# serycjon/WOFT

Hardware: AMD Instinct MI355X
Metric: tracked frames/sec at 1080p, 12 RAFT iters; flow EPE vs reference (higher is better)
Workload: dtype bf16x3 (split-bf16 MFMA operands emulating fp32, fp32 accumulate)

## Files before the change

woft_amd/csrc/conv_1x1_band.hip:

```cpp
#include "conv_1x1_tile.h"
#include "lookup_blocks.h"

int woft_conv_check(const woft_conv_params& p);

namespace {

struct BlockRows {
    int py0, px0, hf, wf;
    __device__ __forceinline__ int64_t operator()(int row) const {
        const int y = py0 + (row >> 3), x = px0 + (row & 7);
        return (y < hf && x < wf) ? (int64_t)y * wf + x : -1;
    }
};

template <int TERMS>
struct GeomBand {
    using G = Geom1x1<TERMS, 2>;
    static constexpr int R = 4, NW = 2 * R + 1, N2 = NW * NW, WS = NW + 1, LEVELS = 4;
    static constexpr int RING = 4;
    static constexpr int RS = WOFT_BAND_LD + 4;
    static constexpr int HR = 6, PLD = HR * RS;
    static constexpr int RING_ELEMS = RING * G::A_ELEMS;
    static constexpr int WIN_ELEMS = 64 * PLD * 2;
    static constexpr int SMEM_ELEMS = RING_ELEMS + WIN_ELEMS;
    static_assert(SMEM_ELEMS >= G::STAGE_ELEMS && SMEM_ELEMS >= Geom1x1<TERMS, 1>::SMEM_ELEMS, "one LDS array for every phase");
    static_assert((RING_ELEMS * 2) % 16 == 0, "the windows start 16-byte aligned");
};

template <int TERMS>
__global__ __launch_bounds__(256, 2) void conv1x1_band_kernel(const woft_conv_params pa, const woft_conv_params pb,
                                                              const woft_lookup_band_params bp, const int split) {
    using GB = GeomBand<TERMS>;
    using G = Geom1x1<TERMS, 2>;
    constexpr int NP = G::NP, TM = G::TM, TN = 2, A_PLANE = G::A_PLANE, A_ELEMS = G::A_ELEMS, WCOLS = G::WCOLS;
    constexpr int R = GB::R, NW = GB::NW, WS = GB::WS, RS = GB::RS, PLD = GB::PLD, NT = 256, NB = 4, NCHUNK = 11;
    constexpr int STEP_ELEMS = NP * 2 * 64 * 8;
    __shared__ __attribute__((aligned(16))) __bf16 smem[GB::SMEM_ELEMS];
    __shared__ int s_ox[GB::LEVELS][64], s_oy[GB::LEVELS][64];
    __shared__ float s_fx[GB::LEVELS][64], s_fy[GB::LEVELS][64];

    if ((int)blockIdx.x >= split) {
        int m_tile, n_tile;
        woft::tile_of_block((int)blockIdx.x - split, m_tiles_1x1(pb), pb.cout_pad / 128, m_tile, n_tile);
        tile_1x1<TERMS, 1, true, 4, 4>(pb, m_tile, n_tile, smem);
        return;
    }
    const woft_lookup_otf_params& p = bp.otf;
    __bf16* const ring = smem;
    float* const Wl = (float*)(smem + GB::RING_ELEMS);

    const int tid = threadIdx.x;
    const int lane = tid & 63;
    const int wave = __builtin_amdgcn_readfirstlane(tid >> 6);
    const int r32 = lane & 31, hh = lane >> 5;
    const int tiles_x = (p.wf + 7) / 8;
    int tile;
    {
        const int q = split / 8, rr = split % 8, xcd = blockIdx.x % 8, idx = blockIdx.x / 8;
        tile = (xcd < rr ? xcd * (q + 1) : rr * (q + 1) + (xcd - rr) * q) + idx;
    }
    const int px0 = (tile % tiles_x) * 8, py0 = (tile / tiles_x) * 8;

    const __bf16* wstream[TN];
#pragma unroll
    for (int j = 0; j < TN; ++j) wstream[j] = (const __bf16*)pa.wgt_frag + (int64_t)(wave * TN + j) * NCHUNK * STEP_ELEMS + lane * 8;
    bf16x8 bq[NB][TN][NP];
    auto fetch_b = [&](int step, auto slot_tag) {
        constexpr int slot = decltype(slot_tag)::value;
        const int s = step < 2 * NCHUNK ? step : 2 * NCHUNK - 1;
        const int off = (s >> 1) * STEP_ELEMS + (s & 1) * 512;
#pragma unroll
        for (int j = 0; j < TN; ++j)
#pragma unroll
            for (int pl = 0; pl < NP; ++pl) bq[slot][j][pl] = *(const bf16x8*)(wstream[j] + off + pl * 1024);
    };
    [&]<int... S>(std::integer_sequence<int, S...>) {
        (fetch_b(S, std::integral_constant<int, S>{}), ...);
    }(std::make_integer_sequence<int, NB - 1>{});

    int ok = 1;
    {
        const int y = py0 + (lane >> 3), x = px0 + (lane & 7);
        const bool cvalid = tid < 64 && y < p.hf && x < p.wf;
        if (cvalid) {
            const int64_t i = (int64_t)y * p.wf + x;
            const float cx = p.coords[i * 2], cy = p.coords[i * 2 + 1];
#pragma unroll
            for (int l = 0; l < GB::LEVELS; ++l) {
                const float sc = 1.0f / (float)(1 << l);
                const float xs = cx * sc, ys = cy * sc;
                float flx = floorf(xs), fly = floorf(ys);
                s_fx[l][tid] = xs - flx;
                s_fy[l][tid] = ys - fly;
                flx = fminf(fmaxf(flx, -1.0e6f), 1.0e6f);
                fly = fminf(fmaxf(fly, -1.0e6f), 1.0e6f);
                const int m = WOFT_BAND_M(l);
                const int ox = (int)flx - (x >> l) + m, oy = (int)fly - (y >> l) + m;
                ok &= (ox >= 0 && ox <= 2 * m && oy >= 0 && oy <= 2 * m) ? 1 : 0;
                s_ox[l][tid] = ox;
                s_oy[l][tid] = oy;
            }
        } else if (tid < 64) {
#pragma unroll
            for (int l = 0; l < GB::LEVELS; ++l) {
                s_fx[l][tid] = s_fy[l][tid] = 0.f;
                s_ox[l][tid] = s_oy[l][tid] = 0;
            }
        }
    }
    const bool hit = __builtin_amdgcn_readfirstlane(__syncthreads_and(ok)) != 0;

    constexpr int ROWS = 16 + 14 + 12 + 12;
    f32x4 pc[GB::HR];
    auto load_half = [&](auto l_tag, auto h_tag) __attribute__((always_inline)) {
        constexpr int l = decltype(l_tag)::value, half = decltype(h_tag)::value;
        constexpr int NR = half == 0 ? 6 : 5, R0 = half == 0 ? 0 : 5;
        constexpr int roff = l == 0 ? 0 : (l == 1 ? 16 : (l == 2 ? 30 : 42));
        static_assert(64 * NR * 4 == NR * NT, "NR pieces per thread");
#pragma unroll
        for (int k = 0; k < NR; ++k) {
            const int it = tid + k * NT;
            const int pix = it / (4 * NR), rem = it - pix * (4 * NR);
            const int gy = py0 + (pix >> 3), gx = px0 + (pix & 7);
            pc[k] = f32x4{0.f, 0.f, 0.f, 0.f};
            if (gy < p.hf && gx < p.wf) {
                const int ox = s_ox[l][pix];
                pc[k] = *(const f32x4*)(bp.band + (((int64_t)gy * p.wf + gx) * ROWS + roff + ox + R0) * WOFT_BAND_LD + rem * 4);
            }
        }
    };
    auto store_half = [&](auto h_tag) __attribute__((always_inline)) {
        constexpr int half = decltype(h_tag)::value;
        constexpr int NR = half == 0 ? 6 : 5;
#pragma unroll
        for (int k = 0; k < NR; ++k) {
            const int it = tid + k * NT;
            const int pix = it / (4 * NR), rem = it - pix * (4 * NR);
            *(f32x4*)(Wl + pix * PLD + (rem >> 2) * RS + (rem & 3) * 4) = pc[k];
        }
    };
    auto sample = [&](auto l_tag, int pix, int c, int lrow) __attribute__((always_inline)) {
        constexpr int l = decltype(l_tag)::value;
        const int gy = py0 + (pix >> 3), gx = px0 + (pix & 7);
        if (gy >= p.hf || gx >= p.wf) return;
        const float fx = s_fx[l][pix], fy = s_fy[l][pix];
        const float* cq = Wl + pix * PLD + lrow * RS + s_oy[l][pix];
        float h[WS];
#pragma unroll
        for (int j = 0; j < WS; ++j) h[j] = cq[j] * (1.f - fx) + cq[RS + j] * fx;
        float o[12];
#pragma unroll
        for (int j = 0; j < NW; ++j) o[j] = h[j] * (1.f - fy) + h[j + 1] * fy;
        o[9] = o[10] = o[11] = 0.f;
        const int ch0 = l * GB::N2 + c * NW;
#pragma unroll
        for (int g = 0; g < 3; ++g) {
            const f32x4 val = {o[4 * g], o[4 * g + 1], o[4 * g + 2], o[4 * g + 3]};
            const bf16x4 hi = cvt16<TERMS>(val);
            bf16x4 lo = hi;
            if (NP == 2) lo = __builtin_convertvector(val - widen_bf16x4(hi), bf16x4);
#pragma unroll
            for (int e = 0; e < 4; ++e) {
                if (4 * g + e >= NW) continue;
                const int ch = ch0 + 4 * g + e;
                __bf16* a = ring + ((ch >> 5) & (GB::RING - 1)) * A_ELEMS + pix * LDB + (ch & 31);
                a[0] = hi[e];
                if (NP == 2) a[A_PLANE] = lo[e];
            }
        }
    };
    const int row = tid >> 2, v = tid & 3;
    const int64_t mrow = BlockRows{py0, px0, p.hf, p.wf}(row);
    auto fill_chunk = [&](int chunk) __attribute__((always_inline)) {
        const f32x4 zero = {0.f, 0.f, 0.f, 0.f};
        f32x4 rh[2] = {zero, zero};
        if (mrow >= 0) {
            const uint32_t off = (uint32_t)mrow * (uint32_t)pa.cs0 + (uint32_t)(chunk * BK + 8 * v);
            rh[0] = *(const f32x4*)(pa.in0 + off);
            rh[1] = *(const f32x4*)(pa.in0 + off + 4);
        }
        bf16x4 hi[2], lo[2];
#pragma unroll
        for (int e = 0; e < 2; ++e) {
            hi[e] = cvt16<TERMS>(rh[e]);
            if (NP == 2) lo[e] = __builtin_convertvector(rh[e] - widen_bf16x4(hi[e]), bf16x4);
        }
        __bf16* As = ring + (chunk & (GB::RING - 1)) * A_ELEMS;
        *(bf16x8*)(As + row * LDB + 8 * v) = __builtin_shufflevector(hi[0], hi[1], 0, 1, 2, 3, 4, 5, 6, 7);
        if (NP == 2) *(bf16x8*)(As + A_PLANE + row * LDB + 8 * v) = __builtin_shufflevector(lo[0], lo[1], 0, 1, 2, 3, 4, 5, 6, 7);
    };

    f32x16 acc[TM][TN];
#pragma unroll
    for (int i = 0; i < TM; ++i)
#pragma unroll
        for (int j = 0; j < TN; ++j)
#pragma unroll
            for (int r = 0; r < 16; ++r) acc[i][j][r] = 0.f;
    const int a_off = r32 * LDB + hh * 8;
    auto run_chunk = [&](auto c_tag) __attribute__((always_inline)) {
        constexpr int c = decltype(c_tag)::value;
        const __bf16* As = ring + (c & (GB::RING - 1)) * A_ELEMS;
        bf16x8 aq[2][TM][NP];
#pragma unroll
        for (int s2 = 0; s2 < 2; ++s2)
#pragma unroll
            for (int i = 0; i < TM; ++i)
#pragma unroll
                for (int pl = 0; pl < NP; ++pl) aq[s2][i][pl] = *(const bf16x8*)(As + a_off + i * 32 * LDB + pl * A_PLANE + s2 * 16);
        [&]<int... S2>(std::integer_sequence<int, S2...>) {
            ([&] {
                constexpr int s2 = S2, slot = (2 * c + s2) % NB;
                fetch_b(2 * c + s2 + NB - 1, std::integral_constant<int, (2 * c + s2 + NB - 1) % NB>{});
                __builtin_amdgcn_sched_barrier(0);
                if (NP == 2) {
#pragma unroll
                    for (int j = 0; j < TN; ++j)
#pragma unroll
                        for (int i = 0; i < TM; ++i) acc[i][j] = mma16<TERMS>(aq[s2][i][NP - 1], bq[slot][j][0], acc[i][j]);
#pragma unroll
                    for (int j = 0; j < TN; ++j)
#pragma unroll
                        for (int i = 0; i < TM; ++i) acc[i][j] = mma16<TERMS>(aq[s2][i][0], bq[slot][j][NP - 1], acc[i][j]);
                }
#pragma unroll
                for (int j = 0; j < TN; ++j)
#pragma unroll
                    for (int i = 0; i < TM; ++i) acc[i][j] = mma16<TERMS>(aq[s2][i][0], bq[slot][j][0], acc[i][j]);
                __builtin_amdgcn_sched_barrier(0);
            }(), ...);
        }(std::make_integer_sequence<int, 2>{});
    };

    if (hit) load_half(std::integral_constant<int, 0>{}, std::integral_constant<int, 0>{});
    auto level = [&](auto l_tag) __attribute__((always_inline)) {
        constexpr int l = decltype(l_tag)::value;
        constexpr int c_first = l == 0 ? 0 : (l == 1 ? 2 : (l == 2 ? 5 : 7));
        constexpr int c_last = l == 0 ? 1 : (l == 1 ? 4 : (l == 2 ? 6 : 10));
        static_assert(c_last == (l == 3 ? NCHUNK - 1 : ((l + 1) * GB::N2) / BK - 1) && c_last - c_first < GB::RING, "ring of four chunk tiles");
        if (hit) {
            store_half(std::integral_constant<int, 0>{});
            __syncthreads();
            load_half(l_tag, std::integral_constant<int, 1>{});
            if (l == 3) {
                __bf16* As = ring + ((NCHUNK - 1) & (GB::RING - 1)) * A_ELEMS + row * LDB;
                const bf16x4 z4 = __builtin_bit_cast(bf16x4, (uint64_t)0);
#pragma unroll
                for (int pl = 0; pl < NP; ++pl) {
                    if (v == 0) *(bf16x4*)(As + pl * A_PLANE + 4) = z4;
                    else *(bf16x8*)(As + pl * A_PLANE + 8 * v) = __builtin_shufflevector(z4, z4, 0, 1, 2, 3, 4, 5, 6, 7);
                }
            }
            for (int it = tid; it < 64 * 5; it += NT) {
                const int pix = it / 5, c = it - pix * 5;
                sample(l_tag, pix, c, c);
            }
            __syncthreads();
            store_half(std::integral_constant<int, 1>{});
            __syncthreads();
            if constexpr (l + 1 < GB::LEVELS) load_half(std::integral_constant<int, l + 1>{}, std::integral_constant<int, 0>{});
            sample(l_tag, tid >> 2, 5 + (tid & 3), tid & 3);
        } else {
            __syncthreads();
#pragma unroll
            for (int c = c_first; c <= c_last; ++c) fill_chunk(c);
        }
        __syncthreads();
        [&]<int... C>(std::integer_sequence<int, C...>) {
            (run_chunk(std::integral_constant<int, c_first + C>{}), ...);
        }(std::make_integer_sequence<int, c_last - c_first + 1>{});
    };
    level(std::integral_constant<int, 0>{});
    level(std::integral_constant<int, 1>{});
    level(std::integral_constant<int, 2>{});
    level(std::integral_constant<int, 3>{});
    __syncthreads();
    woft::conv_epilogue_t<TM, TN, G::BM, WCOLS, G::ST>(pa, acc, (float*)smem + wave * G::ST * woft::STAGE_FLOATS,
                                                        BlockRows{py0, px0, p.hf, p.wf}, 0, 0, wave, lane, tile);
}

}

extern "C" int woft_conv1x1_band(const woft_conv_params* c1, const woft_conv_params* f1, const woft_lookup_band_params* bp,
                                 void* stream) {
    if (c1 == nullptr || bp == nullptr || bp->band == nullptr) return WOFT_EINVAL;
    const woft_lookup_otf_params& o = bp->otf;
    if (o.radius != 4 || o.k != 256 || o.levels != 4 || (o.terms != 1 && o.terms != 3) || o.coords == nullptr || o.out == nullptr ||
        o.hf <= 0 || o.wf <= 0 || o.need != nullptr || o.ablate != 0)
        return WOFT_EINVAL;
    if ((o.roi_y0 | o.roi_x0 | o.roi_h | o.roi_w | o.smp_y0 | o.smp_x0 | o.smp_h | o.smp_w) != 0) return WOFT_EINVAL;
    for (const woft_conv_params* q : {c1, f1}) {
        if (q == nullptr) continue;
        if (woft_conv_check(*q) != WOFT_OK) return WOFT_EINVAL;
        const woft_conv_params& p = *q;
        if (p.halo != 16 || p.precision < 1 || p.precision > 3 || p.precision != c1->precision) return WOFT_EINVAL;
        if (p.stride != 1 || p.ho != p.h || p.wo != p.w || p.taps_x != 1) return WOFT_EINVAL;
        if (p.wgt_frag == nullptr || p.stat_sum != nullptr || p.in_norm != 0 || p.wh0_lookup != nullptr) return WOFT_EINVAL;
        if (p.epi == WOFT_EPI_FLOWHEAD || p.epi == WOFT_EPI_WH_MEAN || p.epi == WOFT_EPI_CTX) return WOFT_EINVAL;
        if ((p.roi_y0 | p.roi_x0 | p.roi_h | p.roi_w) != 0) return WOFT_EINVAL;
        const int64_t cs_max = (p.in1 != nullptr && p.cs1 > p.cs0) ? p.cs1 : p.cs0;
        if ((int64_t)p.n_img * p.h * p.w * cs_max >= (1ll << 31)) return WOFT_EINVAL;
    }
    if (c1->flat || c1->taps_y != 1 || c1->pad_y != 0 || c1->pad_x != 0 || c1->tile_n != 256 || c1->cin_pad != 352 ||
        c1->cout_pad != 256 || c1->in1 != nullptr || c1->n_img != 1 || c1->h != o.hf || c1->w != o.wf)
        return WOFT_EINVAL;
    if (c1->in0 != o.out || c1->cs0 != o.ldo || o.ldo < 352) return WOFT_EINVAL;
    if (f1 != nullptr && (!f1->flat || f1->cin_pad != 32 || f1->tile_n != 128 || 2 * f1->pad_y + 1 != f1->taps_y ||
                          f1->cout_pad % 128 != 0))
        return WOFT_EINVAL;
    const int split = ((o.hf + 7) / 8) * ((o.wf + 7) / 8);
    const int64_t extra = f1 != nullptr ? (int64_t)m_tiles_1x1(*f1) * (f1->cout_pad / 128) : 0;
    dim3 grid((unsigned)(split + extra));
    hipStream_t s = (hipStream_t)stream;
    const woft_conv_params& pb = f1 != nullptr ? *f1 : *c1;
    switch (c1->precision) {
        case 1: woft_launch(0, conv1x1_band_kernel<3>, grid, dim3(256), 0, s, *c1, pb, *bp, split); break;
        case 2: woft_launch(0, conv1x1_band_kernel<1>, grid, dim3(256), 0, s, *c1, pb, *bp, split); break;
        default: woft_launch(0, conv1x1_band_kernel<16>, grid, dim3(256), 0, s, *c1, pb, *bp, split); break;
    }
    return woft_launch_status();
}
```

Before: 130.9.

## Remap band window loads and sampling to one pixel per thread quad

Band-window loads and LDS stores now use a fixed row/quarter mapping per thread (pixel = tid>>2, quarter = tid&3) instead of per-iteration div/mod over pixels. Sampling is re-split so each thread of the quad samples whole rows plus a three-way split of row 4, which removes the loop over 320 items and its idle tail. Per-pixel fx/fy/oy are loaded once per level, and a 31→0 chunk-boundary split handles writes that cross ring tiles. Compile-time-gated timing stamps (WOFT_C1BAND_PROBE) are added but are off by default.

```diff
diff --git a/woft_amd/csrc/conv_1x1_band.hip b/woft_amd/csrc/conv_1x1_band.hip
--- a/woft_amd/csrc/conv_1x1_band.hip
+++ b/woft_amd/csrc/conv_1x1_band.hip
@@ -2,6 +2,19 @@
 #include "lookup_blocks.h"
 
 int woft_conv_check(const woft_conv_params& p);
+
+#ifdef WOFT_C1BAND_PROBE
+#define C1B_STAMPS 46
+#define C1B_STAMP(i, clock)                                      \
+    do {                                                         \
+        __builtin_amdgcn_sched_barrier(0);                       \
+        if (lane == 0) s_stamp[wave][i] = (uint32_t)(clock);     \
+        __builtin_amdgcn_sched_barrier(0);                       \
+    } while (0)
+#else
+#define C1B_STAMP(i, clock) do {} while (0)
+#endif
+#define C1B_TIME(i) C1B_STAMP(i, __builtin_amdgcn_s_memtime())
 
 namespace {
 
@@ -33,11 +46,14 @@
     using GB = GeomBand<TERMS>;
     using G = Geom1x1<TERMS, 2>;
     constexpr int NP = G::NP, TM = G::TM, TN = 2, A_PLANE = G::A_PLANE, A_ELEMS = G::A_ELEMS, WCOLS = G::WCOLS;
-    constexpr int R = GB::R, NW = GB::NW, WS = GB::WS, RS = GB::RS, PLD = GB::PLD, NT = 256, NB = 4, NCHUNK = 11;
+    constexpr int R = GB::R, NW = GB::NW, RS = GB::RS, PLD = GB::PLD, NT = 256, NB = 4, NCHUNK = 11;
     constexpr int STEP_ELEMS = NP * 2 * 64 * 8;
     __shared__ __attribute__((aligned(16))) __bf16 smem[GB::SMEM_ELEMS];
     __shared__ int s_ox[GB::LEVELS][64], s_oy[GB::LEVELS][64];
     __shared__ float s_fx[GB::LEVELS][64], s_fy[GB::LEVELS][64];
+#ifdef WOFT_C1BAND_PROBE
+    __shared__ uint32_t s_stamp[4][C1B_STAMPS];
+#endif
 
     if ((int)blockIdx.x >= split) {
         int m_tile, n_tile;
@@ -52,6 +68,8 @@
     const int tid = threadIdx.x;
     const int lane = tid & 63;
     const int wave = __builtin_amdgcn_readfirstlane(tid >> 6);
+    C1B_STAMP(44, __builtin_amdgcn_s_memrealtime());
+    C1B_TIME(0);
     const int r32 = lane & 31, hh = lane >> 5;
     const int tiles_x = (p.wf + 7) / 8;
     int tile;
@@ -110,67 +128,60 @@
     }
     const bool hit = __builtin_amdgcn_readfirstlane(__syncthreads_and(ok)) != 0;
 
+    const int row = tid >> 2, v = tid & 3;
+    const int64_t mrow = BlockRows{py0, px0, p.hf, p.wf}(row);
+
     constexpr int ROWS = 16 + 14 + 12 + 12;
     f32x4 pc[GB::HR];
     auto load_half = [&](auto l_tag, auto h_tag) __attribute__((always_inline)) {
         constexpr int l = decltype(l_tag)::value, half = decltype(h_tag)::value;
         constexpr int NR = half == 0 ? 6 : 5, R0 = half == 0 ? 0 : 5;
         constexpr int roff = l == 0 ? 0 : (l == 1 ? 16 : (l == 2 ? 30 : 42));
-        static_assert(64 * NR * 4 == NR * NT, "NR pieces per thread");
-#pragma unroll
-        for (int k = 0; k < NR; ++k) {
-            const int it = tid + k * NT;
-            const int pix = it / (4 * NR), rem = it - pix * (4 * NR);
-            const int gy = py0 + (pix >> 3), gx = px0 + (pix & 7);
-            pc[k] = f32x4{0.f, 0.f, 0.f, 0.f};
-            if (gy < p.hf && gx < p.wf) {
-                const int ox = s_ox[l][pix];
-                pc[k] = *(const f32x4*)(bp.band + (((int64_t)gy * p.wf + gx) * ROWS + roff + ox + R0) * WOFT_BAND_LD + rem * 4);
-            }
+        static_assert(64 * 4 == NT && NR <= GB::HR, "a quarter of every row of one pixel per thread");
+#pragma unroll
+        for (int k = 0; k < NR; ++k) pc[k] = f32x4{0.f, 0.f, 0.f, 0.f};
+        if (mrow >= 0) {
+            const float* src = bp.band + (mrow * ROWS + roff + s_ox[l][row] + R0) * WOFT_BAND_LD + v * 4;
+#pragma unroll
+            for (int k = 0; k < NR; ++k) pc[k] = *(const f32x4*)(src + k * WOFT_BAND_LD);
         }
     };
     auto store_half = [&](auto h_tag) __attribute__((always_inline)) {
         constexpr int half = decltype(h_tag)::value;
         constexpr int NR = half == 0 ? 6 : 5;
 #pragma unroll
-        for (int k = 0; k < NR; ++k) {
-            const int it = tid + k * NT;
-            const int pix = it / (4 * NR), rem = it - pix * (4 * NR);
-            *(f32x4*)(Wl + pix * PLD + (rem >> 2) * RS + (rem & 3) * 4) = pc[k];
-        }
-    };
-    auto sample = [&](auto l_tag, int pix, int c, int lrow) __attribute__((always_inline)) {
-        constexpr int l = decltype(l_tag)::value;
-        const int gy = py0 + (pix >> 3), gx = px0 + (pix & 7);
-        if (gy >= p.hf || gx >= p.wf) return;
-        const float fx = s_fx[l][pix], fy = s_fy[l][pix];
-        const float* cq = Wl + pix * PLD + lrow * RS + s_oy[l][pix];
-        float h[WS];
-#pragma unroll
-        for (int j = 0; j < WS; ++j) h[j] = cq[j] * (1.f - fx) + cq[RS + j] * fx;
-        float o[12];
-#pragma unroll
-        for (int j = 0; j < NW; ++j) o[j] = h[j] * (1.f - fy) + h[j + 1] * fy;
-        o[9] = o[10] = o[11] = 0.f;
-        const int ch0 = l * GB::N2 + c * NW;
-#pragma unroll
-        for (int g = 0; g < 3; ++g) {
+        for (int k = 0; k < NR; ++k) *(f32x4*)(Wl + row * PLD + k * RS + v * 4) = pc[k];
+    };
+    auto sample = [&](auto l_tag, auto n_tag, int c, int lrow, int j0, float fx, float fy, int oy) __attribute__((always_inline)) {
+        constexpr int l = decltype(l_tag)::value, NJ = decltype(n_tag)::value, NG = (NJ + 3) / 4;
+        const float* cq = Wl + row * PLD + lrow * RS + oy + j0;
+        float h[NJ + 1];
+#pragma unroll
+        for (int j = 0; j <= NJ; ++j) h[j] = cq[j] * (1.f - fx) + cq[RS + j] * fx;
+        float o[4 * NG];
+#pragma unroll
+        for (int j = 0; j < NJ; ++j) o[j] = h[j] * (1.f - fy) + h[j + 1] * fy;
+#pragma unroll
+        for (int j = NJ; j < 4 * NG; ++j) o[j] = 0.f;
+        const int ch0 = l * GB::N2 + c * NW + j0, kw = BK - (ch0 & (BK - 1));
+        const int a0 = ((ch0 >> 5) & (GB::RING - 1)) * A_ELEMS + row * LDB + (ch0 & (BK - 1));
+        const int a1 = (((ch0 >> 5) + 1) & (GB::RING - 1)) * A_ELEMS + row * LDB - kw;
+#pragma unroll
+        for (int g = 0; g < NG; ++g) {
             const f32x4 val = {o[4 * g], o[4 * g + 1], o[4 * g + 2], o[4 * g + 3]};
             const bf16x4 hi = cvt16<TERMS>(val);
             bf16x4 lo = hi;
             if (NP == 2) lo = __builtin_convertvector(val - widen_bf16x4(hi), bf16x4);
 #pragma unroll
             for (int e = 0; e < 4; ++e) {
-                if (4 * g + e >= NW) continue;
-                const int ch = ch0 + 4 * g + e;
-                __bf16* a = ring + ((ch >> 5) & (GB::RING - 1)) * A_ELEMS + pix * LDB + (ch & 31);
+                if (4 * g + e >= NJ) continue;
+                const int k = 4 * g + e;
+                __bf16* a = ring + (k < kw ? a0 : a1) + k;
                 a[0] = hi[e];
                 if (NP == 2) a[A_PLANE] = lo[e];
             }
         }
     };
-    const int row = tid >> 2, v = tid & 3;
-    const int64_t mrow = BlockRows{py0, px0, p.hf, p.wf}(row);
     auto fill_chunk = [&](int chunk) __attribute__((always_inline)) {
         const f32x4 zero = {0.f, 0.f, 0.f, 0.f};
         f32x4 rh[2] = {zero, zero};
@@ -233,15 +244,23 @@
     };
 
     if (hit) load_half(std::integral_constant<int, 0>{}, std::integral_constant<int, 0>{});
+    C1B_TIME(1);
     auto level = [&](auto l_tag) __attribute__((always_inline)) {
         constexpr int l = decltype(l_tag)::value;
+        constexpr std::integral_constant<int, NW> whole{};
+        [[maybe_unused]] constexpr int T0 = 2 + 10 * l;
         constexpr int c_first = l == 0 ? 0 : (l == 1 ? 2 : (l == 2 ? 5 : 7));
         constexpr int c_last = l == 0 ? 1 : (l == 1 ? 4 : (l == 2 ? 6 : 10));
         static_assert(c_last == (l == 3 ? NCHUNK - 1 : ((l + 1) * GB::N2) / BK - 1) && c_last - c_first < GB::RING, "ring of four chunk tiles");
         if (hit) {
+            C1B_TIME(T0);
             store_half(std::integral_constant<int, 0>{});
+            C1B_TIME(T0 + 1);
             __syncthreads();
+            C1B_TIME(T0 + 2);
             load_half(l_tag, std::integral_constant<int, 1>{});
+            const float fx = s_fx[l][row], fy = s_fy[l][row];
+            const int oy = s_oy[l][row];
             if (l == 3) {
                 __bf16* As = ring + ((NCHUNK - 1) & (GB::RING - 1)) * A_ELEMS + row * LDB;
                 const bf16x4 z4 = __builtin_bit_cast(bf16x4, (uint64_t)0);
@@ -251,32 +270,46 @@
                     else *(bf16x8*)(As + pl * A_PLANE + 8 * v) = __builtin_shufflevector(z4, z4, 0, 1, 2, 3, 4, 5, 6, 7);
                 }
             }
-            for (int it = tid; it < 64 * 5; it += NT) {
-                const int pix = it / 5, c = it - pix * 5;
-                sample(l_tag, pix, c, c);
-            }
+            if (mrow >= 0) {
+                sample(l_tag, whole, v, v, 0, fx, fy, oy);
+                if (v < 3) sample(l_tag, std::integral_constant<int, 3>{}, 4, 4, 3 * v, fx, fy, oy);
+            }
+            C1B_TIME(T0 + 3);
             __syncthreads();
+            C1B_TIME(T0 + 4);
             store_half(std::integral_constant<int, 1>{});
+            C1B_TIME(T0 + 5);
             __syncthreads();
+            C1B_TIME(T0 + 6);
             if constexpr (l + 1 < GB::LEVELS) load_half(std::integral_constant<int, l + 1>{}, std::integral_constant<int, 0>{});
-            sample(l_tag, tid >> 2, 5 + (tid & 3), tid & 3);
+            if (mrow >= 0) sample(l_tag, whole, 5 + v, v, 0, fx, fy, oy);
+            C1B_TIME(T0 + 7);
         } else {
             __syncthreads();
 #pragma unroll
             for (int c = c_first; c <= c_last; ++c) fill_chunk(c);
         }
         __syncthreads();
+        C1B_TIME(T0 + 8);
         [&]<int... C>(std::integer_sequence<int, C...>) {
             (run_chunk(std::integral_constant<int, c_first + C>{}), ...);
         }(std::make_integer_sequence<int, c_last - c_first + 1>{});
+        C1B_TIME(T0 + 9);
     };
     level(std::integral_constant<int, 0>{});
     level(std::integral_constant<int, 1>{});
     level(std::integral_constant<int, 2>{});
     level(std::integral_constant<int, 3>{});
     __syncthreads();
+    C1B_TIME(42);
     woft::conv_epilogue_t<TM, TN, G::BM, WCOLS, G::ST>(pa, acc, (float*)smem + wave * G::ST * woft::STAGE_FLOATS,
                                                         BlockRows{py0, px0, p.hf, p.wf}, 0, 0, wave, lane, tile);
+    C1B_TIME(43);
+    C1B_STAMP(45, __builtin_amdgcn_s_memrealtime());
+#ifdef WOFT_C1BAND_PROBE
+    if (hit && lane < C1B_STAMPS && px0 + wave < p.wf)
+        ((uint32_t*)p.out)[((int64_t)py0 * p.wf + px0 + wave) * p.ldo + lane] = s_stamp[wave][lane];
+#endif
 }
 
 }
```

Measured after the change: 131.5 (median of 3 runs). About the same (+0.4%).
